# swanhong/matrix-fhe-lattigo

Hardware: AMD Instinct MI355X
Metric: forward-NTT/s at N=2^16, 16 RNS limbs; achieved HBM GB/s vs peak (higher is better)
Workload: dtype u64

## Files before the change

### matrix-fhe-lattigo_amd/csrc/engine.hip

```cpp
#include <hip/hip_runtime.h>
#include <cstdio>
#include <cstdarg>
#include <cstring>
#include <vector>
#include <new>
#include "../../include/ringhip.h"
#include "hostmath.hpp"
#include "ntt_kernels.hip.hpp"
#include "vec_kernels.hip.hpp"
#include "stream_kernels.hip.hpp"
#include "ntt_kernels_asm.hip.hpp"
#include "ntt3n_kernels_asm.hip.hpp"
#include "engine_internal.hpp"

static thread_local char g_err[512] = "";
int rh_fail(int code, const char* fmt, ...) {
  va_list ap; va_start(ap, fmt); vsnprintf(g_err, sizeof(g_err), fmt, ap); va_end(ap);
  return code;
}
extern "C" const char* rh_last_error(void) { return g_err; }

static thread_local hipStream_t tl_stream = nullptr;
static thread_local bool tl_has_stream = false;
static thread_local u64* tl_ws = nullptr;
// ... 416 lines not shown
  } else {
    if (phase != 1) {
      if (r->asm_tile && S1 == 0 && r->inv_scale && r->one_pass && phase == 0) {
        if (nt) ntt_inv_onepass_asm<0, true><<<rows, 256, (size_t)LDS_WORDS * 8, st>>>(in, out, r->d_twk_inv + toff, r->d_tw_inv + toff, r->d_lastw + limb0, c, Lrows, Ls, Lso, 1);
        else ntt_inv_onepass_asm<0, false><<<rows, 256, (size_t)LDS_WORDS * 8, st>>>(in, out, r->d_twk_inv + toff, r->d_tw_inv + toff, r->d_lastw + limb0, c, Lrows, Ls, Lso, 1);
        return rh_launch_ok("ntt (N = 4096, inverse)");
      }
      if (r->asm_tile && (S1 > 0 || !r->inv_scale) && nt) ntt_inv_tile_asm<true><<<tiles, 256, 0, st>>>(in, out, r->d_twk_inv + toff, c, Lrows, logN, npoly, Ls, Lso);
      else if (r->asm_tile && (S1 > 0 || !r->inv_scale)) ntt_inv_tile_asm<false><<<tiles, 256, 0, st>>>(in, out, r->d_twk_inv + toff, c, Lrows, logN, npoly, Ls, Lso);
      else ntt_inv_tile<<<tiles, 256, 0, st>>>(in, out, r->d_twk_inv + toff, c, Lrows, logN, (S1 == 0 && r->inv_scale) ? 1 : 0, npoly, Ls, Lso);
    }
    const bool acols = phase != 2 && r->asm_cols && r->asm_tile && r->inv_scale;
    if (S1 == 4 && acols && nt) ntt_inv_cols_asm<4, true><<<dim3(rows * 16), 256, 0, st>>>(out, r->d_tw_inv + toff, r->d_lastw + limb0, c, Lrows, Lso);
    else if (S1 == 3 && acols && nt) ntt_inv_cols_asm<3, true><<<dim3(rows * 16), 256, 0, st>>>(out, r->d_tw_inv + toff, r->d_lastw + limb0, c, Lrows, Lso);
    else if (S1 == 2 && acols && nt) ntt_inv_cols_asm<2, true><<<dim3(rows * 16), 256, 0, st>>>(out, r->d_tw_inv + toff, r->d_lastw + limb0, c, Lrows, Lso);
    else if (S1 == 4 && acols) ntt_inv_cols_asm<4><<<dim3(rows * 16), 256, 0, st>>>(out, r->d_tw_inv + toff, r->d_lastw + limb0, c, Lrows, Lso);
    else if (S1 == 3 && acols) ntt_inv_cols_asm<3><<<dim3(rows * 16), 256, 0, st>>>(out, r->d_tw_inv + toff, r->d_lastw + limb0, c, Lrows, Lso);
    else if (S1 == 2 && acols) ntt_inv_cols_asm<2><<<dim3(rows * 16), 256, 0, st>>>(out, r->d_tw_inv + toff, r->d_lastw + limb0, c, Lrows, Lso);
    else if (S1 > 0 && phase != 2) launch_inv_cols(S1, dim3(rows * 16), st, out, r->d_tw_inv + toff, r->d_lastw + limb0, c, Lrows, logN, r->inv_scale ? 1 : 0, Lso);
  }
  return rh_launch_ok("ntt");
}

template <int S1>
static void launch_fused(rh_ring* r, const u64* in1, u64* out1, unsigned n1, u64* data2, unsigned n2, int npoly2,
                         size_t toff, const LimbConsts* c, int Lrows) {
  const unsigned grid = n1 > n2 ? n1 : n2;
  hipStream_t st = rh_stream(r);
  constexpr bool has_acols = S1 >= 2 && S1 <= 4;
  if constexpr (has_acols) {
    if (r->asm_tile && r->asm_cols) {
      if (r->nt_streams) ntt_fwd_fused_asm<S1, true, true><<<grid, 256, 0, st>>>(in1, out1, n1, data2, n2, npoly2, r->d_tw_fwd + toff, r->d_twk_fwd + toff, c, Lrows, r->logN);
      else ntt_fwd_fused_asm<S1, true, false><<<grid, 256, 0, st>>>(in1, out1, n1, data2, n2, npoly2, r->d_tw_fwd + toff, r->d_twk_fwd + toff, c, Lrows, r->logN);
      return;
    }
  }
  if (r->asm_tile)
    ntt_fwd_fused_asm<S1, false><<<grid, 256, 0, st>>>(in1, out1, n1, data2, n2, npoly2, r->d_tw_fwd + toff, r->d_twk_fwd + toff, c, Lrows, r->logN);
  else
    ntt_fwd_fused<ShoupPolicy, S1><<<grid, 256, 0, st>>>(in1, out1, n1, data2, n2, npoly2, r->d_tw_fwd + toff, r->d_twk_fwd + toff,
                                                      c, Lrows, r->logN, 1);
}

struct NttSeg { const u64* in; u64* out; int npoly; };
static int std_ntt_fwd_pipelined_segs(rh_ring* r, const NttSeg* segs, int nseg, int Lrows, int limb0, int chunk) {
  (void)hipGetLastError();
  const int N = r->N, S1 = r->logN - LT;
  const size_t toff = (size_t)limb0 * N, stride = (size_t)Lrows * N;
  const LimbConsts* c = r->d_consts + limb0;
  std::vector<NttSeg> spans;
  for (int k = 0; k < nseg; ++k)
    for (int p = 0; p < segs[k].npoly; p += chunk)
      spans.push_back(NttSeg{segs[k].in + (size_t)p * stride, segs[k].out + (size_t)p * stride, segs[k].npoly - p < chunk ? segs[k].npoly - p : chunk});
  const int nspans = (int)spans.size();
// ... 3 lines not shown
    const u64* i1 = j < nspans ? spans[j].in : nullptr; u64* o1 = j < nspans ? spans[j].out : nullptr; u64* d2 = j >= 1 ? spans[j - 1].out : nullptr;
    switch (S1) {
      case 1: launch_fused<1>(r, i1, o1, n1, d2, n2, n2p, toff, c, Lrows); break;
      case 2: launch_fused<2>(r, i1, o1, n1, d2, n2, n2p, toff, c, Lrows); break;
      case 3: launch_fused<3>(r, i1, o1, n1, d2, n2, n2p, toff, c, Lrows); break;
      case 4: launch_fused<4>(r, i1, o1, n1, d2, n2, n2p, toff, c, Lrows); break;
      case 5: launch_fused<5>(r, i1, o1, n1, d2, n2, n2p, toff, c, Lrows); break;
    }
  }
  return rh_launch_ok("ntt_fwd_fused");
}
static int std_ntt_fwd_pipelined(rh_ring* r, const u64* in, u64* out, int npoly, int Lrows, int limb0, int chunk) {
  const NttSeg seg{in, out, npoly};
  return std_ntt_fwd_pipelined_segs(r, &seg, 1, Lrows, limb0, chunk);
}

template <int S1>
static void launch_inv_fused(rh_ring* r, const u64* in1, const u64* in1b, u64* out1, unsigned n1, int npoly1, u64* data2, unsigned n2,
                             size_t toff, int limb0, const LimbConsts* c, int Lrows) {
  const unsigned grid = n1 > n2 ? n1 : n2;
  hipStream_t st = rh_stream(r);
  constexpr bool has_acols = S1 >= 2 && S1 <= 4;
  const bool acols = has_acols && r->asm_cols;
  if (in1b) {
    const tw2* lw = r->d_lastw_r + limb0;
    if constexpr (has_acols) {
      if (acols) { ntt_inv_fused_asm<S1, true, true><<<grid, 256, 0, st>>>(in1, in1b, out1, n1, npoly1, data2, n2, r->d_twk_inv + toff, r->d_tw_inv + toff, lw, c, Lrows, r->logN); return; }
    }
    ntt_inv_fused_asm<S1, false, true><<<grid, 256, 0, st>>>(in1, in1b, out1, n1, npoly1, data2, n2, r->d_twk_inv + toff, r->d_tw_inv + toff, lw, c, Lrows, r->logN);
    return;
  }
  const tw2* lw = r->d_lastw + limb0;
  if constexpr (has_acols) {
    if (acols && !r->nt_streams) { ntt_inv_fused_asm<S1, true, false, false><<<grid, 256, 0, st>>>(in1, nullptr, out1, n1, npoly1, data2, n2, r->d_twk_inv + toff, r->d_tw_inv + toff, lw, c, Lrows, r->logN); return; }
    if (acols) { ntt_inv_fused_asm<S1, true, false><<<grid, 256, 0, st>>>(in1, nullptr, out1, n1, npoly1, data2, n2, r->d_twk_inv + toff, r->d_tw_inv + toff, lw, c, Lrows, r->logN); return; }
  }
  ntt_inv_fused_asm<S1, false, false><<<grid, 256, 0, st>>>(in1, nullptr, out1, n1, npoly1, data2, n2, r->d_twk_inv + toff, r->d_tw_inv + toff, lw, c, Lrows, r->logN);
}
static int std_ntt_inv_pipelined(rh_ring* r, const u64* in, u64* out, int npoly, int Lrows, int limb0, int chunk, const u64* in_b = nullptr) {
  (void)hipGetLastError();
  const int N = r->N, S1 = r->logN - LT;
  const size_t toff = (size_t)limb0 * N, stride = (size_t)Lrows * N;
  const LimbConsts* c = (in_b ? r->d_consts_r : r->d_consts) + limb0;
  const int nspans = (npoly + chunk - 1) / chunk;
  for (int j = 0; j <= nspans; ++j) {
    const int p1 = j * chunk, n1p = j < nspans ? ((npoly - p1 < chunk) ? npoly - p1 : chunk) : 0;
    const int p2 = (j - 1) * chunk, n2p = j >= 1 ? ((npoly - p2 < chunk) ? npoly - p2 : chunk) : 0;
    const unsigned n1 = ((unsigned)n1p * Lrows) << S1, n2 = (unsigned)n2p * Lrows * 16;
    const u64* i1 = in + (size_t)p1 * stride; u64* o1 = out + (size_t)p1 * stride; u64* d2 = out + (size_t)p2 * stride;
    const u64* ib = in_b ? in_b + (size_t)p1 * stride : nullptr;
    switch (S1) {
      case 1: launch_inv_fused<1>(r, i1, ib, o1, n1, n1p, d2, n2, toff, limb0, c, Lrows); break;
      case 2: launch_inv_fused<2>(r, i1, ib, o1, n1, n1p, d2, n2, toff, limb0, c, Lrows); break;
      case 3: launch_inv_fused<3>(r, i1, ib, o1, n1, n1p, d2, n2, toff, limb0, c, Lrows); break;
      case 4: launch_inv_fused<4>(r, i1, ib, o1, n1, n1p, d2, n2, toff, limb0, c, Lrows); break;
      case 5: launch_inv_fused<5>(r, i1, ib, o1, n1, n1p, d2, n2, toff, limb0, c, Lrows); break;
// ... 472 lines not shown
  if (npoly < 0) return rh_fail(RH_ERR_ARG, "polymul: npoly < 0");
  if (a == b) return rh_fail(RH_ERR_ARG, "polymul: a and b must be different blocks (both are transformed in place)");
  const int S1 = r->logN - LT;
  if (r->kind != RH_RING_STANDARD || S1 < 1 || S1 > 5 || !r->asm_tile) return rh_fail(RH_ERR_UNSUPPORTED, "polymul: standard rings with 2^13 <= N <= 2^17 and the hand-scheduled tile bodies");
  const int Lrows = level + 1;
  const unsigned rows = (unsigned)npoly * (unsigned)Lrows;
  if (rows == 0) return RH_OK;
  (void)hipSetDevice(r->device);
  hipStream_t st = rh_stream(r);
  int chunk = r->chunk_polys;
  if (chunk < 0) { const int c = r->auto_span_rows / Lrows > 0 ? r->auto_span_rows / Lrows : 1; chunk = npoly > c ? c : 0; }
  if (chunk > 0 && npoly > chunk) {
    (void)hipGetLastError();
    const int nspans = (npoly + chunk - 1) / chunk;
    const size_t stride = (size_t)Lrows * r->N;
    const bool nt = r->nt_streams != 0;
    auto span = [&](int j, int* n) { const int p0 = j * chunk; *n = (j < 0 || j >= nspans) ? 0 : (npoly - p0 < chunk ? npoly - p0 : chunk); return (size_t)(j < 0 ? 0 : p0) * stride; };
    for (int j = 0; j < nspans + 2; ++j) {
      int p1, p2, p3;
      const size_t o1 = span(j, &p1), o2 = span(j - 1, &p2), o3 = span(j - 2, &p3);
      const unsigned n1 = (unsigned)p1 * Lrows * 16, n2 = ((unsigned)p2 * Lrows) << S1, n3 = (unsigned)p3 * Lrows * 16;
      const unsigned grid = n1 > n2 ? (n1 > n3 ? n1 : n3) : (n2 > n3 ? n2 : n3);
      if (!grid) continue;
#define RH_PM_FUSED(S) do { if (nt) ntt_polymul_fused_asm<S, true><<<grid, 256, 0, st>>>(a + o1, b + o1, n1, a + o2, b + o2, out + o2, n2, p2, out + o3, n3, r->d_tw_fwd, r->d_twk_fwd, \
                                                                                          r->d_twk_inv, r->d_tw_inv, r->d_lastw_r, r->d_consts_r, Lrows, r->logN);                          \
                            else ntt_polymul_fused_asm<S, false><<<grid, 256, 0, st>>>(a + o1, b + o1, n1, a + o2, b + o2, out + o2, n2, p2, out + o3, n3, r->d_tw_fwd, r->d_twk_fwd,      \
                                                                                       r->d_twk_inv, r->d_tw_inv, r->d_lastw_r, r->d_consts_r, Lrows, r->logN); } while (0)
      switch (S1) { case 1: RH_PM_FUSED(1); break; case 2: RH_PM_FUSED(2); break; case 3: RH_PM_FUSED(3); break; case 4: RH_PM_FUSED(4); break; default: RH_PM_FUSED(5); break; }
#undef RH_PM_FUSED
    }
    return rh_launch_ok("polymul (pipelined)");
  }
  if (int rc = std_ntt_launch_span(r, a, a, npoly, Lrows, 0, false, false, 1)) return rc;
  if (int rc = std_ntt_launch_span(r, b, b, npoly, Lrows, 0, false, false, 1)) return rc;
  (void)hipGetLastError();
  if (rh_stream_grid(r, rows).nt) ntt_polymul_tile_asm<true><<<rows << S1, 256, 0, st>>>(a, b, out, r->d_twk_fwd, r->d_twk_inv, r->d_consts_r, Lrows, r->logN, npoly);
  else ntt_polymul_tile_asm<false><<<rows << S1, 256, 0, st>>>(a, b, out, r->d_twk_fwd, r->d_twk_inv, r->d_consts_r, Lrows, r->logN, npoly);
  const bool nt = rh_stream_grid(r, rows).nt;
  if (S1 >= 2 && S1 <= 4 && r->asm_cols) {
#define RH_PM_COLS(S) do { if (nt) ntt_inv_cols_asm<S, true><<<dim3(rows * 16), 256, 0, st>>>(out, r->d_tw_inv, r->d_lastw_r, r->d_consts_r, Lrows, 0); \
                           else ntt_inv_cols_asm<S, false><<<dim3(rows * 16), 256, 0, st>>>(out, r->d_tw_inv, r->d_lastw_r, r->d_consts_r, Lrows, 0); } while (0)
    if (S1 == 4) RH_PM_COLS(4); else if (S1 == 3) RH_PM_COLS(3); else RH_PM_COLS(2);
#undef RH_PM_COLS
  } else launch_inv_cols(S1, dim3(rows * 16), st, out, r->d_tw_inv, r->d_lastw_r, r->d_consts_r, Lrows, r->logN, 1);
  return rh_launch_ok("polymul");
}

// ... 21 lines not shown
  return rh_rescale_reserve(r, npoly);
}

extern "C" int rh_ring_set_tuning(rh_ring* r, const char* key, long value) {
  if (!r || !key) return rh_fail(RH_ERR_ARG, "set_tuning: null argument");
  if (!strcmp(key, "chunk_polys")) { r->chunk_polys = (int)value; return RH_OK; }
  if (!strcmp(key, "asm_tile")) { r->asm_tile = value != 0; return RH_OK; }
  if (!strcmp(key, "auto_span_rows")) { if (value < 1) return rh_fail(RH_ERR_ARG, "auto_span_rows must be >= 1"); r->auto_span_rows = (int)value; return RH_OK; }
  if (!strcmp(key, "fuse_submul")) { r->fuse_submul = (int)value; return RH_OK; }
  if (!strcmp(key, "digit_pipeline")) { r->digit_pipeline = (int)value; return RH_OK; }
  if (!strcmp(key, "fuse_ci")) { r->fuse_ci = (int)value; return RH_OK; }
  if (!strcmp(key, "perm_inv_shape")) { r->perm_inv_shape = (int)value; return RH_OK; }
  if (!strcmp(key, "perm_fwd_shape")) { r->perm_fwd_shape = (int)value; return RH_OK; }
  if (!strcmp(key, "fuse3n")) { r->fuse3n = (int)value; return RH_OK; }
  if (!strcmp(key, "ntt3n_block_order")) {
    if (r->kind != RH_RING_3N) return rh_fail(RH_ERR_ARG, "ntt3n_block_order: not a 3N ring");
    r->block_order3n = value != 0;
    return RH_OK;
  }
  if (!strcmp(key, "asm_cols")) { r->asm_cols = (int)value; return RH_OK; }
  if (!strcmp(key, "ks_small_rows")) { if (value < 0) return rh_fail(RH_ERR_ARG, "ks_small_rows must be >= 0"); r->ks_small_rows = (int)value; return RH_OK; }
  if (!strcmp(key, "pair_submul")) { r->pair_submul = value != 0; return RH_OK; }
  if (!strcmp(key, "one_pass")) { r->one_pass = value != 0; return RH_OK; }
  if (!strcmp(key, "nt_streams")) {
    if (value < 0 || value > 2) return rh_fail(RH_ERR_ARG, "nt_streams must be 0, 1 or 2 (got %ld)", value);
    r->nt_streams = (int)value; if (r->kind == RH_RING_3N) rh_ring3n_set_nt_streams(r, (int)value); return RH_OK;
  }
  return rh_fail(RH_ERR_ARG, "set_tuning: unknown key %s", key);
}

static int slot_acquire(rh_ring* r, RhHostSlot** out) {
  {
    std::lock_guard<std::mutex> lk(r->slot_mu);
    if (!r->free_slots.empty()) { *out = r->free_slots.back(); r->free_slots.pop_back(); return RH_OK; }
  }
  RhHostSlot* sl = new (std::nothrow) RhHostSlot();
  if (!sl) return rh_fail(RH_ERR_NOMEM, "out of host memory");
  sl->words = (size_t)r->N * (r->kind == RH_RING_3N ? 2 : 1);
  if (hipStreamCreateWithFlags(&sl->stream, hipStreamNonBlocking) != hipSuccess) { delete sl; return rh_fail(RH_ERR_DEVICE, "hipStreamCreate failed"); }
  if (hipMalloc((void**)&sl->buf, sl->words * 8) != hipSuccess) { (void)hipStreamDestroy(sl->stream); delete sl; return rh_fail(RH_ERR_NOMEM, "hipMalloc(host-limb scratch) failed"); }
  std::lock_guard<std::mutex> lk(r->slot_mu);
  r->all_slots.push_back(sl);
  *out = sl;
  return RH_OK;
}
static void slot_release(rh_ring* r, RhHostSlot* sl) {
// ... 250 lines not shown
```

### matrix-fhe-lattigo_amd/csrc/engine_internal.hpp

```cpp
#pragma once
#include <hip/hip_runtime.h>
#include <vector>
#include <mutex>
#include <atomic>
#include <cstdint>
#include "../../include/ringhip.h"
#include "ring_types.hip.hpp"

#define RH_MAX_LIMBS 64

int rh_fail(int code, const char* fmt, ...);

inline bool rh_nt_policy(int nt_streams, size_t bytes, size_t threshold) { return nt_streams == 2 || (nt_streams == 1 && bytes >= threshold); }

struct rh_ring3n_state;
struct CiFold { tw2 f, b; };

struct rh_ring {
  int device = 0, kind = 0, N = 0, logN = 0, L = 0;
  hipStream_t stream = nullptr;
  std::vector<uint64_t> moduli, mred, bred, ninv, roots_fwd, roots_bwd, omega3n;
  std::vector<LimbConsts> hconsts;
  LimbConsts* d_consts = nullptr;
  tw2* d_tw_fwd = nullptr;
// ... 12 lines not shown
  std::vector<struct RhPolySlot*> free_poly_slots, all_poly_slots;
  std::recursive_mutex mu;
  rh_ring3n_state* s3n = nullptr;
  std::vector<void*> rescale_tables;
  u64* d_rs[2] = {nullptr, nullptr}; size_t rs_words[2] = {0, 0};
  u64* d_rows = nullptr; size_t rows_words = 0;
  std::atomic<long> stats_rows_direct{0}, stats_rows_compacted{0};
  int fuse_submul = 1;
  int fuse_ci = 1;
  int digit_pipeline = 1;
  int perm_fwd_shape = 44;
  int perm_inv_shape = 44;
  int fuse3n = 1;
  int block_order3n = 0;
  int asm_cols = 1;
  bool asm_tile = true;
  bool inv_scale = true;
  int auto_span_rows = 2048;
  int ks_small_rows = 512;
  bool pair_submul = true;
  bool one_pass = true;
  bool one_pass_ready = false;
  int nt_streams = 1;
  int chunk_polys = -1;
};

int rh_launch_ok(const char* what);
struct RhStreamGrid { dim3 grid; int nt; };
unsigned rh_stream_chunks(const rh_ring* r);
RhStreamGrid rh_stream_grid(const rh_ring* r, unsigned rows);
inline RhStreamGrid rh_stream_begin(const rh_ring* r, unsigned rows) {
  (void)hipSetDevice(r->device);
  (void)hipGetLastError();
  return rh_stream_grid(r, rows);
}
int rh_scheme_args(const rh_ring* r, int level, int npoly, unsigned kinds, int n_multiple, const char* who);
int rh_comps3(const void* in0, const void* in1, const void* in2, const void* out0, const void* out1, const void* out2, const char* who);
struct RhScalars { u64 a[RH_MAX_LIMBS]; u64 b[RH_MAX_LIMBS]; };
int rh_pack_scalars(const rh_ring* r, int level, const u64* a, const u64* b, bool mont, RhScalars* s, const char* who, const char* noun = "scalar");

struct RhHostSlot { hipStream_t stream = nullptr; u64* buf = nullptr; size_t words = 0; };
hipStream_t rh_stream(const rh_ring* r);
u64* rh_ws_override(size_t words);
struct RhCallScope {
  RhCallScope(hipStream_t st, u64* ws = nullptr, size_t ws_words = 0);
  ~RhCallScope();
// ... 16 lines not shown
int rh_std_ntt_fwd_blocks_small(rh_ring* r, u64* data, size_t block_stride, int nblocks, int Ls, const int* gap0, const int* gap_len,
                                rh_ring* r2, u64* data2, size_t block_stride2, int nblocks2, int Ls2, int npoly, bool lazy_out);
bool rh_can_intt_limb_strided(const rh_ring* r);
int rh_std_intt_limb_strided(rh_ring* r, const u64* in, int in_rows, int limb, u64* out, int npoly);
bool rh_can_fuse_submul(const rh_ring* r);
int rh_std_ntt_submul_launch(rh_ring* r, u64* buf, int npoly, int Lrows, int limb0, const u64* y, int y_rows, u64* out, int out_rows,
                             const u64* scalars_host, bool cols_done = false, const u64* z = nullptr, int z_rows = 0);
int rh_std_ntt_submul_launch_pair(rh_ring* r, u64* buf, int npoly, int Lrows, const u64* y0, const u64* y1, int y_rows, u64* out0, u64* out1, int out_rows,
                                  const u64* scalars_host, const u64* z0, const u64* z1, int z_rows);
int rh_std_ntt_expand_cols_launch(rh_ring* r, const u64* tmp, u64* buf, int npoly, int Lrows, const void* table_dev, int mode, u64 qL);
int rh_vec_launch(rh_ring* r, int opcode, const u64* p1, const u64* p2, u64* p3, int npoly, int Lrows, int limb0,
                  const u64* s0, const u64* s1, int rows1 = 0, int rows2 = 0, int rows3 = 0, int half = 0);
int rh_std_intt_rows(rh_ring* r, const u64* in, int in_rows, u64* out, int out_rows, int npoly, int Lrows);
int rh_std_upload_tables(rh_ring* r, const std::vector<tw2>& fs, const std::vector<tw2>& is, const std::vector<u64>* mont,
                         const std::vector<tw2>& lastw);
int rh_upload_consts(rh_ring* r, const std::vector<LimbConsts>& hc);
void rh_rescale_teardown(rh_ring* r);
int rh_rescale_reserve(rh_ring* r, int npoly);
int rh_ring3n_reserve(rh_ring* r, int npoly);
void rh_3n_launch_layer(bool inverse, int S1, unsigned nblocks, hipStream_t st, const u64* in, u64* out, const N3Layer& a, int nt_streams);
int rh_ring3n_setup(rh_ring* r, std::vector<LimbConsts>& hc);
void rh_ring3n_teardown(rh_ring* r);
void rh_ring3n_set_nt_streams(rh_ring* r, int policy);
int rh_ring3n_ntt_launch(rh_ring* r, const u64* in, u64* out, int npoly, int Lrows, int limb0, bool inverse, bool block_order = false);
int rh_ring3n_reorder_launch(rh_ring* r, const u64* in, u64* out, int npoly, int Lrows, bool to_reference);

struct rh_bext;
rh_ring* rh_bext_ringQ(rh_bext* be);
rh_ring* rh_bext_ringP(rh_bext* be);
int rh_bext_scratch(rh_bext* be, int which, size_t words, u64** out);
std::recursive_mutex& rh_bext_mutex(rh_bext* be);
struct RhBextGuard {
  std::unique_lock<std::recursive_mutex> lk; RhCallScope sc;
  explicit RhBextGuard(rh_bext* be) : lk(rh_bext_mutex(be)), sc(rh_stream(rh_bext_ringQ(be))) {}
};
int rh_bext_moddown_ntt_add(rh_bext* be, int levelQ, int levelP, const u64* p1Q, const u64* p1P, u64* p2Q, int npoly, const u64* addend);
int rh_bext_moddown_ntt_pair(rh_bext* be, int levelQ, int levelP, const u64* q0, const u64* q1, const u64* p1P, u64* out0, u64* out1,
                             int npoly, const u64* add0, const u64* add1);
```

### matrix-fhe-lattigo_amd/csrc/ntt3n.hip

```cpp
#include <hip/hip_runtime.h>
#include <vector>
#include <cstring>
#include "engine_internal.hpp"
#include "hostmath.hpp"

struct rh_ring3n_state {
  int a = 0, b = 0, nb = 0, n2 = 0, log_n2 = 0;
  rh_ring* sub = nullptr;
  Limb3N* d_l3 = nullptr;
  tw2* d_r3_fwd = nullptr;
  tw2* d_r3_inv = nullptr;
  std::vector<int> r3_off;
  int r3_stride = 0;
  int* d_rank = nullptr;
  int* d_block_of_rank = nullptr;
  u64* d_tmp = nullptr; size_t tmp_words = 0;
};

RH_DEV u64 add4(u64 x, u64 y, u64 q4) { return csub(x + y, q4); }
RH_DEV u64 sub4(u64 x, u64 y, u64 q4) { return csub(x + q4 - y, q4); }

__global__ void __launch_bounds__(256)
ntt3n_split_fwd(const u64* in, u64* out, int N, const Limb3N* __restrict__ l3, const LimbConsts* __restrict__ consts, int L) {
  const u32 row = blockIdx.x, limb = row % (u32)L;
// ... 558 lines not shown
      ntt3n_perm_inv<<<dim3(rows, chunks(N)), 256, 0, st>>>(in, tmp, N, nb, s->log_n2, s->d_block_of_rank);
    const int S1sub = s->sub ? s->log_n2 - 12 : 0;
    const bool fuse = s->b == 1 && s->sub && r->fuse3n && S1sub >= 1 && S1sub <= 3;
    if (s->sub) {
      if (int rc = rh_std_ntt_launch(s->sub, tmp, tmp, npoly, Lrows * nb, limb0 * nb, true, false, fuse ? 2 : 0)) return rc;
    }
    if (fuse) {
      const tw2* stw = s->sub->d_tw_inv + ((size_t)limb0 * nb << s->log_n2);
      const dim3 g(rows * 16);
      launch_cols_post_inv(r, S1sub, g, st, tmp, out, N, r3i + s->r3_off[1], s->r3_stride, l3, c, Lrows, stw, s->log_n2);
    } else if (s->b == 1) {
      ntt3n_post_b1_inv<<<dim3(rows, chunks(N / 6)), 256, 0, st>>>(tmp, out, N, r3i + s->r3_off[1], s->r3_stride, l3, c, Lrows);
    } else {
      int cnt = nb / 3, step = s->n2;
      for (int l = s->b; l >= 1; --l, cnt /= 3, step *= 3)
        ntt3n_radix3_inv<<<dim3(rows, chunks(cnt * step)), 256, 0, st>>>(tmp, N, step, cnt, r3i + s->r3_off[l], s->r3_stride, l3, c, Lrows);
      ntt3n_split_inv<<<dim3(rows, chunks(N / 2)), 256, 0, st>>>(tmp, out, N, l3, c, Lrows);
    }
  }
  return rh_launch_ok("3N transform");
}

void rh_ring3n_set_nt_streams(rh_ring* r, int policy) { if (r->s3n && r->s3n->sub) r->s3n->sub->nt_streams = policy; }

int rh_ring3n_reserve(rh_ring* r, int npoly) { return ensure_tmp(r->s3n, (size_t)npoly * r->L * r->N); }
```

### matrix-fhe-lattigo_amd/csrc/ntt_kernels.hip.hpp

```cpp
#pragma once
#include "modarith.hip.hpp"

#include "ring_types.hip.hpp"

struct ShoupPolicy {
  typedef tw2 tw_t;
  u64 q, nq, q4;
  RH_DEV void init(const LimbConsts& c) { q = c.q; nq = c.nq; q4 = 4 * c.q; }
  RH_DEV void fwd(u64& U, u64& V, const tw_t& w, bool ) const {
    u64 u = csub(U, q4);
    u64 X = shoup_mul_acc(V, w.w, w.wp, nq, u);
    V = ((u << 1) + q4) - X;
    U = X;
  }
  RH_DEV void inv(u64& U, u64& V, const tw_t& w) const {
    u64 d = U + q4 - V;
    U = csub(U + V, q4);
    V = shoup_mul(d, w.w, w.wp, nq);
  }
  RH_DEV u64 fwd_final(u64 x, bool canonical) const { return canonical ? canon8(x, q) : x; }
};

struct MontPolicy {
  typedef u64 tw_t;
// ... 261 lines not shown
  const RescaleLimb l = T[limb];
  ShoupPolicy p; p.init(consts[limb]);
  u64 x[R];
#pragma unroll
  for (int k = 0; k < R; ++k) {
    u64 t = tmp[((size_t)poly << logN) + col + ((size_t)k << LT)];
    if (mode == 1) t = cred(t + ((qL - 1) >> 1), qL) + l.s;
    x[k] = bred_add(t, l.q, l.bred0);
  }
#pragma unroll
  for (int s = 0; s < S1; ++s) {
    const int h = R >> (s + 1);
#pragma unroll
    for (int g = 0; g < (1 << s); ++g) {
      tw2 w = tw[(1 << s) + g];
#pragma unroll
      for (int e = 0; e < h; ++e) p.fwd(x[g * 2 * h + e], x[g * 2 * h + e + h], w, false);
    }
  }
#pragma unroll
  for (int k = 0; k < R; ++k) out[base + ((size_t)k << LT)] = x[k];
}

template <class P, int S1>
__global__ void __launch_bounds__(256)
ntt_fwd_fused(const u64* in1, u64* out1, unsigned n1, u64* data2, unsigned n2, int npoly2,
              const typename P::tw_t* __restrict__ twn, const typename P::tw_t* __restrict__ twk,
              const LimbConsts* __restrict__ consts, int L, int logN, int canonical) {
  __shared__ u64 lds[LDS_WORDS];
  if (blockIdx.x < n1) fwd_cols_body<P, S1>(blockIdx.x, in1, out1, twn, consts, L, logN);
  if (blockIdx.x < n2) fwd_tile_body<P>(lds, blockIdx.x, data2, data2, twk, consts, L, logN, canonical, npoly2, L);
}

template <int S1>
RH_DEV void inv_cols_body(const u32 b, u64* data, const tw2* __restrict__ twn, const tw2* __restrict__ lastw,
                          const LimbConsts* __restrict__ consts, int L, int logN, int scale, int Ls = 0) {
  constexpr int R = 1 << S1;
  const u32 limb = b % (u32)L;
  const u32 r = b / (u32)L;
  const u32 cb = r & 15;
  const u32 poly = r >> 4;
  const size_t base = (((size_t)poly * (Ls ? Ls : L) + limb) << logN) + cb * 256 + threadIdx.x;
  const tw2* tw = twn + ((size_t)limb << logN);
  const LimbConsts c = consts[limb];
  ShoupPolicy p; p.init(c);
  u64 x[R];
// ... 116 lines not shown
```

### matrix-fhe-lattigo_amd/csrc/ntt_kernels_asm.hip.hpp

```cpp
#pragma once
#include "ring_types.hip.hpp"
#include "ntt_kernels.hip.hpp"
#include "ntt_tile_asm.inc"
#include "ntt_ci_asm.inc"


template <bool LAZY = false, bool NT = false>
RH_DEV void fwd_tile_asm_body(u64* lds, const u32 b, const u64* in, u64* out, const tw2* __restrict__ twk,
                              const LimbConsts* __restrict__ consts, int L, int logN, int npoly, int Ls = 0, u32 gap0 = 0, u32 gap_len = 0, int Lso = 0) {
  if (Ls == 0) Ls = L;
  if (Lso == 0) Lso = Ls;
  const u32 lrow = b % (u32)L;
  const u32 limb = lrow + (lrow >= gap0 ? gap_len : 0u);
  const u32 r = b / (u32)L;
  const u32 poly = r % (u32)npoly;
  const u32 tile = r / (u32)npoly;
  const size_t base = (((size_t)poly * Ls + limb) << logN) + ((size_t)tile << LT);
  const u64 pin = uni64((u64)(size_t)(in + base));
  const u64 pout = uni64((u64)(size_t)(out + (((size_t)poly * Lso + limb) << logN) + ((size_t)tile << LT)));
  const u64 tw = uni64((u64)(size_t)(twk + ((size_t)limb << logN) + ((size_t)tile << LT)));
  const u64 q = uni64(consts[limb].q);
  const u64 nq = (u64)0 - q, nq2 = (u64)0 - 2 * q, nq4 = (u64)0 - 4 * q, q4 = 4 * q;
  const u32 lds_off = uni32((u32)(size_t)lds);
  const u32 tid = threadIdx.x;
// ... 106 lines not shown
  const u64 q = uni64(consts[limb].q);
  const u64 sw = uni64(sc.w[limb]), sp = uni64(sc.wp[limb]);
  const u64 nq = (u64)0 - q, nq2 = (u64)0 - 2 * q, nq4 = (u64)0 - 4 * q, q4 = 4 * q, q2 = 2 * q;
  const u32 lds_off = uni32((u32)(size_t)lds);
  const u32 tid = threadIdx.x;
#define RH_SUBMUL_ADD_ASM(BODY)                                                                                                      \
  asm volatile(BODY : : [tid] "v"(tid), [lds] "s"(lds_off), [pin] "s"(pin), [pout] "s"(pout), [py] "s"(py), [pz] "s"(pz), [tw] "s"(tw),     \
               [twlo] "s"((u32)(size_t)tw), [twhi] "s"((u32)((size_t)tw >> 32)), [nq0] "s"((u32)nq), [nq1] "s"((u32)(nq >> 32)),            \
               [nq] "s"(nq), [nq2] "s"(nq2), [nq4] "s"(nq4), [q4] "s"(q4), [q2] "s"(q2), [sw0] "s"((u32)sw), [sw1] "s"((u32)(sw >> 32)),    \
               [sp0] "s"((u32)sp), [sp1] "s"((u32)(sp >> 32)) : NTT_TILE_ASM_CLOBBERS)
#define RH_SUBMUL_ASM(BODY)                                                                                                          \
  asm volatile(BODY : : [tid] "v"(tid), [lds] "s"(lds_off), [pin] "s"(pin), [pout] "s"(pout), [py] "s"(py), [tw] "s"(tw),                   \
               [twlo] "s"((u32)(size_t)tw), [twhi] "s"((u32)((size_t)tw >> 32)), [nq0] "s"((u32)nq), [nq1] "s"((u32)(nq >> 32)),            \
               [nq] "s"(nq), [nq2] "s"(nq2), [nq4] "s"(nq4), [q4] "s"(q4), [q2] "s"(q2), [sw0] "s"((u32)sw), [sw1] "s"((u32)(sw >> 32)),    \
               [sp0] "s"((u32)sp), [sp1] "s"((u32)(sp >> 32)) : NTT_TILE_ASM_CLOBBERS)
  if constexpr (ADD && NT) RH_SUBMUL_ADD_ASM(NTT_TILE_SUBMUL_ADD_ASM_BODY_NT);
  else if constexpr (ADD) RH_SUBMUL_ADD_ASM(NTT_TILE_SUBMUL_ADD_ASM_BODY);
  else if constexpr (NT) RH_SUBMUL_ASM(NTT_TILE_SUBMUL_ASM_BODY_NT);
  else RH_SUBMUL_ASM(NTT_TILE_SUBMUL_ASM_BODY);
#undef RH_SUBMUL_ADD_ASM
#undef RH_SUBMUL_ASM
}

template <int S1, bool ASMCOLS = false, bool NT = true>
__global__ void __launch_bounds__(256)
ntt_fwd_fused_asm(const u64* in1, u64* out1, unsigned n1, u64* data2, unsigned n2, int npoly2,
                  const tw2* __restrict__ twn, const tw2* __restrict__ twk, const LimbConsts* __restrict__ consts, int L, int logN) {
  __shared__ u64 lds[LDS_WORDS];
  if (blockIdx.x < n1) fwd_cols_best<S1, ASMCOLS, NT>(blockIdx.x, in1, out1, twn, consts, L, logN);
  if (blockIdx.x < n2) fwd_tile_asm_body<false, NT>(lds, blockIdx.x, data2, data2, twk, consts, L, logN, npoly2);
}

struct GapRows { int L, Ls; u32 gap0, gap_len; };
template <int S1, bool LAZY, bool NT>
__global__ void __launch_bounds__(256)
ntt_fwd_fused_gap_asm(u64* data1, unsigned n1, GapRows g1, u64* data2, unsigned n2, int npoly2, GapRows g2,
                      const tw2* __restrict__ twn, const tw2* __restrict__ twk, const LimbConsts* __restrict__ consts) {
  __shared__ u64 lds[LDS_WORDS];
  if (blockIdx.x < n1) fwd_cols_asm_body<S1, NT>(blockIdx.x, data1, data1, twn, consts, g1.L, g1.Ls, g1.gap0, g1.gap_len);
  if (blockIdx.x < n2) fwd_tile_asm_body<LAZY, NT>(lds, blockIdx.x, data2, data2, twk, consts, g2.L, LT + S1, npoly2, g2.Ls, g2.gap0, g2.gap_len);
}

struct GapBlocks { int L[8]; u32 gap0[8], gap_len[8]; int Ls; };
struct BlockSet { u64* data; size_t stride; const tw2* tw; const LimbConsts* consts; GapBlocks g; int nblocks; };
template <int S1>
__global__ void __launch_bounds__(256)
ntt_fwd_cols_blocks_asm(BlockSet a, BlockSet b, int npoly) {
  const bool first = blockIdx.y < (unsigned)a.nblocks;
  const u32 y = first ? blockIdx.y : blockIdx.y - (unsigned)a.nblocks;
  const GapBlocks& g = first ? a.g : b.g;
  const int L = g.L[y];
// ... 109 lines not shown
  const u64 pin = uni64((u64)(size_t)(a + base)), pin2 = uni64((u64)(size_t)(b2 + base)), pout = uni64((u64)(size_t)(out + base));
  const u64 tw = uni64((u64)(size_t)(twk_fwd + toff)), twi = uni64((u64)(size_t)(twk_inv + toff));
  const u64 q = uni64(consts[limb].q), qinv = uni64(consts[limb].qinv);
  const u64 nq = (u64)0 - q, nq2 = (u64)0 - 2 * q, nq4 = (u64)0 - 4 * q, q4 = 4 * q;
  const u32 lds_off = uni32((u32)(size_t)lds);
  const u32 tid = threadIdx.x;
#define RH_TILE_POLYMUL_ASM(BODY)                                                                                                          \
  asm volatile(BODY : : [tid] "v"(tid), [lds] "s"(lds_off), [pin] "s"(pin), [pin2] "s"(pin2), [pout] "s"(pout), [tw] "s"(tw),               \
               [twlo] "s"((u32)(size_t)tw), [twhi] "s"((u32)((size_t)tw >> 32)), [twi] "s"(twi), [twilo] "s"((u32)(size_t)twi),            \
               [twihi] "s"((u32)((size_t)twi >> 32)), [nq0] "s"((u32)nq), [nq1] "s"((u32)(nq >> 32)), [nq] "s"(nq), [nq2] "s"(nq2),       \
               [nq4] "s"(nq4), [q4] "s"(q4), [q] "s"(q), [q0] "s"((u32)q), [q1] "s"((u32)(q >> 32)), [qi0] "s"((u32)qinv),                 \
               [qi1] "s"((u32)(qinv >> 32)) : NTT_TILE_POLYMUL_ASM_CLOBBERS)
  if constexpr (NT) RH_TILE_POLYMUL_ASM(NTT_TILE_POLYMUL_ASM_BODY_NT);
  else RH_TILE_POLYMUL_ASM(NTT_TILE_POLYMUL_ASM_BODY);
#undef RH_TILE_POLYMUL_ASM
}
template <bool NT = false>
__global__ void __launch_bounds__(256)
ntt_polymul_tile_asm(const u64* a, const u64* b2, u64* out, const tw2* __restrict__ twk_fwd, const tw2* __restrict__ twk_inv,
                     const LimbConsts* __restrict__ consts, int L, int logN, int npoly) {
  __shared__ u64 lds[LDS_WORDS];
  polymul_tile_asm_body<NT>(lds, blockIdx.x, a, b2, out, twk_fwd, twk_inv, consts, L, logN, npoly);
}
template <int S1, bool NT>
__global__ void __launch_bounds__(256)
ntt_polymul_fused_asm(u64* a1, u64* b1, unsigned n1, const u64* a2, const u64* b2, u64* out2, unsigned n2, int npoly2, u64* out3, unsigned n3,
                      const tw2* __restrict__ twn_f, const tw2* __restrict__ twk_f, const tw2* __restrict__ twk_i, const tw2* __restrict__ twn_i,
                      const tw2* __restrict__ lastw_r, const LimbConsts* __restrict__ consts_r, int L, int logN) {
  __shared__ u64 lds[LDS_WORDS];
  const u32 b = blockIdx.x;
  if (b < n1) {
    fwd_cols_best<S1, true, NT>(b, a1, a1, twn_f, consts_r, L, logN);
    fwd_cols_best<S1, true, NT>(b, b1, b1, twn_f, consts_r, L, logN);
  }
  if (b < n2) polymul_tile_asm_body<NT>(lds, b, a2, b2, out2, twk_f, twk_i, consts_r, L, logN, npoly2);
  if (b < n3) {
    if constexpr (has_asm_cols(S1)) inv_cols_asm_body<S1, NT>(b, out3, twn_i, lastw_r, consts_r, L);
    else inv_cols_body<S1>(b, out3, twn_i, lastw_r, consts_r, L, logN, 1);
  }
}

template <int S1, bool ASMCOLS = false, bool MUL = false, bool NT = true>
__global__ void __launch_bounds__(256)
ntt_inv_fused_asm(const u64* in1, const u64* in1b, u64* out1, unsigned n1, int npoly1, u64* data2, unsigned n2,
                  const tw2* __restrict__ twk, const tw2* __restrict__ twn, const tw2* __restrict__ lastw,
                  const LimbConsts* __restrict__ consts, int L, int logN) {
  __shared__ u64 lds[LDS_WORDS];
  if (blockIdx.x < n2) {
    if constexpr (has_asm_cols(S1) && ASMCOLS) inv_cols_asm_body<S1, NT>(blockIdx.x, data2, twn, lastw, consts, L);
    else inv_cols_body<S1>(blockIdx.x, data2, twn, lastw, consts, L, logN, 1);
  }
  if (blockIdx.x < n1) inv_tile_asm_body<MUL, NT>(lds, blockIdx.x, in1, in1b, out1, twk, consts, L, logN, npoly1);
}

struct CiFoldTw { tw2 f, b; };
template <int S1, bool INV>
RH_DEV void cols_ci_asm_body(const u32 b, const u64* in, u64* out, const tw2* __restrict__ twn, const tw2* __restrict__ lastw,
                             const CiFoldTw* __restrict__ fold, const LimbConsts* __restrict__ consts, int L) {
  static_assert(has_asm_cols(S1), "asm column stages exist for S1 = 2..4");
  constexpr int logN = LT + S1;
  const u32 limb = b % (u32)L, rr = b / (u32)L, g = rr & 7;
  const size_t row = ((size_t)(rr >> 3) * L + limb) << logN;
  const size_t offa = row + 256 * g + 1, offb = row + 256 * (15 - g);
  const u64 pina = uni64((u64)(size_t)(in + offa)), pinb = uni64((u64)(size_t)(in + offb));
  const u64 pouta = uni64((u64)(size_t)(out + offa)), poutb = uni64((u64)(size_t)(out + offb));
  const u64 tw = uni64((u64)(size_t)(twn + ((size_t)limb << logN)));
  const u64 q = uni64(consts[limb].q);
  const u64 nq = (u64)0 - q, nq2 = (u64)0 - 2 * q, nq4 = (u64)0 - 4 * q, q4 = 4 * q;
  const tw2 F = INV ? fold[limb].b : fold[limb].f;
  const u64 fw = uni64(F.w), fp = uni64(F.wp);
// ... 250 lines not shown
```

Before: 146,000.

## Spread column-stage units across tile-sized grid in fused NTT kernels

When a fused kernel's column-stage unit count differs from its tile count, the launch grid shrinks to roughly the tile count, with a floor of one eighth of the column units. Each block then loops over a contiguous range of column units before doing at most one tile. This replaces many short-lived blocks that do only column work with fewer blocks that each do more, aiming to balance work per block and cut block scheduling overhead. The cost is lower parallelism and possible tail imbalance. The behaviour is controlled by a new fused_spread knob, which is on by default.

Result: no change. 146,000 (median of 2 runs) (-0.0%).

```diff
diff --git a/matrix-fhe-lattigo_amd/csrc/engine.hip b/matrix-fhe-lattigo_amd/csrc/engine.hip
--- a/matrix-fhe-lattigo_amd/csrc/engine.hip
+++ b/matrix-fhe-lattigo_amd/csrc/engine.hip
@@ -462,6 +462,13 @@
   return rh_launch_ok("ntt");
 }
 
+struct FusedShape { unsigned grid; bool spread; };
+static FusedShape fused_shape(const rh_ring* r, unsigned n_tile, unsigned n_a, unsigned n_b = 0) {
+  const unsigned m = n_a > n_b ? n_a : n_b, all = m > n_tile ? m : n_tile;
+  if (!r->fused_spread || !n_tile || ((!n_a || n_a == n_tile) && (!n_b || n_b == n_tile))) return {all, false};
+  const unsigned least = (m + 7) / 8;
+  return {n_tile > least ? n_tile : least, true};
+}
 template <int S1>
 static void launch_fused(rh_ring* r, const u64* in1, u64* out1, unsigned n1, u64* data2, unsigned n2, int npoly2,
                          size_t toff, const LimbConsts* c, int Lrows) {
@@ -470,6 +477,12 @@
   constexpr bool has_acols = S1 >= 2 && S1 <= 4;
   if constexpr (has_acols) {
     if (r->asm_tile && r->asm_cols) {
+      const FusedShape fs = fused_shape(r, n2, n1);
+      if (fs.spread) {
+        if (r->nt_streams) ntt_fwd_fused_asm<S1, true, true, true><<<fs.grid, 256, 0, st>>>(in1, out1, n1, data2, n2, npoly2, r->d_tw_fwd + toff, r->d_twk_fwd + toff, c, Lrows, r->logN);
+        else ntt_fwd_fused_asm<S1, true, false, true><<<fs.grid, 256, 0, st>>>(in1, out1, n1, data2, n2, npoly2, r->d_tw_fwd + toff, r->d_twk_fwd + toff, c, Lrows, r->logN);
+        return;
+      }
       if (r->nt_streams) ntt_fwd_fused_asm<S1, true, true><<<grid, 256, 0, st>>>(in1, out1, n1, data2, n2, npoly2, r->d_tw_fwd + toff, r->d_twk_fwd + toff, c, Lrows, r->logN);
       else ntt_fwd_fused_asm<S1, true, false><<<grid, 256, 0, st>>>(in1, out1, n1, data2, n2, npoly2, r->d_tw_fwd + toff, r->d_twk_fwd + toff, c, Lrows, r->logN);
       return;
@@ -519,9 +532,11 @@
   hipStream_t st = rh_stream(r);
   constexpr bool has_acols = S1 >= 2 && S1 <= 4;
   const bool acols = has_acols && r->asm_cols;
+  const FusedShape fs = fused_shape(r, n1, n2);
   if (in1b) {
     const tw2* lw = r->d_lastw_r + limb0;
     if constexpr (has_acols) {
+      if (acols && fs.spread) { ntt_inv_fused_asm<S1, true, true, true, true><<<fs.grid, 256, 0, st>>>(in1, in1b, out1, n1, npoly1, data2, n2, r->d_twk_inv + toff, r->d_tw_inv + toff, lw, c, Lrows, r->logN); return; }
       if (acols) { ntt_inv_fused_asm<S1, true, true><<<grid, 256, 0, st>>>(in1, in1b, out1, n1, npoly1, data2, n2, r->d_twk_inv + toff, r->d_tw_inv + toff, lw, c, Lrows, r->logN); return; }
     }
     ntt_inv_fused_asm<S1, false, true><<<grid, 256, 0, st>>>(in1, in1b, out1, n1, npoly1, data2, n2, r->d_twk_inv + toff, r->d_tw_inv + toff, lw, c, Lrows, r->logN);
@@ -529,6 +544,8 @@
   }
   const tw2* lw = r->d_lastw + limb0;
   if constexpr (has_acols) {
+    if (acols && fs.spread && !r->nt_streams) { ntt_inv_fused_asm<S1, true, false, false, true><<<fs.grid, 256, 0, st>>>(in1, nullptr, out1, n1, npoly1, data2, n2, r->d_twk_inv + toff, r->d_tw_inv + toff, lw, c, Lrows, r->logN); return; }
+    if (acols && fs.spread) { ntt_inv_fused_asm<S1, true, false, true, true><<<fs.grid, 256, 0, st>>>(in1, nullptr, out1, n1, npoly1, data2, n2, r->d_twk_inv + toff, r->d_tw_inv + toff, lw, c, Lrows, r->logN); return; }
     if (acols && !r->nt_streams) { ntt_inv_fused_asm<S1, true, false, false><<<grid, 256, 0, st>>>(in1, nullptr, out1, n1, npoly1, data2, n2, r->d_twk_inv + toff, r->d_tw_inv + toff, lw, c, Lrows, r->logN); return; }
     if (acols) { ntt_inv_fused_asm<S1, true, false><<<grid, 256, 0, st>>>(in1, nullptr, out1, n1, npoly1, data2, n2, r->d_twk_inv + toff, r->d_tw_inv + toff, lw, c, Lrows, r->logN); return; }
   }
@@ -1047,7 +1064,12 @@
       const unsigned n1 = (unsigned)p1 * Lrows * 16, n2 = ((unsigned)p2 * Lrows) << S1, n3 = (unsigned)p3 * Lrows * 16;
       const unsigned grid = n1 > n2 ? (n1 > n3 ? n1 : n3) : (n2 > n3 ? n2 : n3);
       if (!grid) continue;
-#define RH_PM_FUSED(S) do { if (nt) ntt_polymul_fused_asm<S, true><<<grid, 256, 0, st>>>(a + o1, b + o1, n1, a + o2, b + o2, out + o2, n2, p2, out + o3, n3, r->d_tw_fwd, r->d_twk_fwd, \
+      const FusedShape fs = fused_shape(r, n2, n1, n3);
+#define RH_PM_FUSED(S) do { if (fs.spread && nt) ntt_polymul_fused_asm<S, true, true><<<fs.grid, 256, 0, st>>>(a + o1, b + o1, n1, a + o2, b + o2, out + o2, n2, p2, out + o3, n3, r->d_tw_fwd, r->d_twk_fwd, \
+                                                                                                       r->d_twk_inv, r->d_tw_inv, r->d_lastw_r, r->d_consts_r, Lrows, r->logN);             \
+                            else if (fs.spread) ntt_polymul_fused_asm<S, false, true><<<fs.grid, 256, 0, st>>>(a + o1, b + o1, n1, a + o2, b + o2, out + o2, n2, p2, out + o3, n3, r->d_tw_fwd, r->d_twk_fwd, \
+                                                                                                       r->d_twk_inv, r->d_tw_inv, r->d_lastw_r, r->d_consts_r, Lrows, r->logN);             \
+                            else if (nt) ntt_polymul_fused_asm<S, true><<<grid, 256, 0, st>>>(a + o1, b + o1, n1, a + o2, b + o2, out + o2, n2, p2, out + o3, n3, r->d_tw_fwd, r->d_twk_fwd, \
                                                                                           r->d_twk_inv, r->d_tw_inv, r->d_lastw_r, r->d_consts_r, Lrows, r->logN);                          \
                             else ntt_polymul_fused_asm<S, false><<<grid, 256, 0, st>>>(a + o1, b + o1, n1, a + o2, b + o2, out + o2, n2, p2, out + o3, n3, r->d_tw_fwd, r->d_twk_fwd,      \
                                                                                        r->d_twk_inv, r->d_tw_inv, r->d_lastw_r, r->d_consts_r, Lrows, r->logN); } while (0)
@@ -1115,6 +1137,10 @@
   if (!strcmp(key, "ks_small_rows")) { if (value < 0) return rh_fail(RH_ERR_ARG, "ks_small_rows must be >= 0"); r->ks_small_rows = (int)value; return RH_OK; }
   if (!strcmp(key, "pair_submul")) { r->pair_submul = value != 0; return RH_OK; }
   if (!strcmp(key, "one_pass")) { r->one_pass = value != 0; return RH_OK; }
+  if (!strcmp(key, "fused_spread")) {
+    if (value < 0 || value > 1) return rh_fail(RH_ERR_ARG, "fused_spread must be 0 or 1 (got %ld)", value);
+    r->fused_spread = (int)value; if (r->kind == RH_RING_3N) rh_ring3n_set_fused_spread(r, (int)value); return RH_OK;
+  }
   if (!strcmp(key, "nt_streams")) {
     if (value < 0 || value > 2) return rh_fail(RH_ERR_ARG, "nt_streams must be 0, 1 or 2 (got %ld)", value);
     r->nt_streams = (int)value; if (r->kind == RH_RING_3N) rh_ring3n_set_nt_streams(r, (int)value); return RH_OK;
diff --git a/matrix-fhe-lattigo_amd/csrc/engine_internal.hpp b/matrix-fhe-lattigo_amd/csrc/engine_internal.hpp
--- a/matrix-fhe-lattigo_amd/csrc/engine_internal.hpp
+++ b/matrix-fhe-lattigo_amd/csrc/engine_internal.hpp
@@ -58,6 +58,7 @@
   bool one_pass = true;
   bool one_pass_ready = false;
   int nt_streams = 1;
+  int fused_spread = 1;
   int chunk_polys = -1;
 };
 
@@ -120,6 +121,7 @@
 int rh_ring3n_setup(rh_ring* r, std::vector<LimbConsts>& hc);
 void rh_ring3n_teardown(rh_ring* r);
 void rh_ring3n_set_nt_streams(rh_ring* r, int policy);
+void rh_ring3n_set_fused_spread(rh_ring* r, int spread);
 int rh_ring3n_ntt_launch(rh_ring* r, const u64* in, u64* out, int npoly, int Lrows, int limb0, bool inverse, bool block_order = false);
 int rh_ring3n_reorder_launch(rh_ring* r, const u64* in, u64* out, int npoly, int Lrows, bool to_reference);
 
diff --git a/matrix-fhe-lattigo_amd/csrc/ntt3n.hip b/matrix-fhe-lattigo_amd/csrc/ntt3n.hip
--- a/matrix-fhe-lattigo_amd/csrc/ntt3n.hip
+++ b/matrix-fhe-lattigo_amd/csrc/ntt3n.hip
@@ -604,5 +604,6 @@
 }
 
 void rh_ring3n_set_nt_streams(rh_ring* r, int policy) { if (r->s3n && r->s3n->sub) r->s3n->sub->nt_streams = policy; }
+void rh_ring3n_set_fused_spread(rh_ring* r, int spread) { if (r->s3n && r->s3n->sub) r->s3n->sub->fused_spread = spread; }
 
 int rh_ring3n_reserve(rh_ring* r, int npoly) { return ensure_tmp(r->s3n, (size_t)npoly * r->L * r->N); }
diff --git a/matrix-fhe-lattigo_amd/csrc/ntt_kernels.hip.hpp b/matrix-fhe-lattigo_amd/csrc/ntt_kernels.hip.hpp
--- a/matrix-fhe-lattigo_amd/csrc/ntt_kernels.hip.hpp
+++ b/matrix-fhe-lattigo_amd/csrc/ntt_kernels.hip.hpp
@@ -307,6 +307,12 @@
   for (int k = 0; k < R; ++k) out[base + ((size_t)k << LT)] = x[k];
 }
 
+RH_DEV u32 fused_div(const u64 p, const u32 G) { return (p >> 32) == 0 ? (u32)p / G : (u32)(p / G); }
+RH_DEV void fused_units(const u32 n, u32& lo, u32& hi) {
+  const u32 b = blockIdx.x, G = gridDim.x;
+  if (n == G) { lo = b; hi = b + 1; return; }
+  lo = fused_div((u64)b * n, G); hi = fused_div((u64)(b + 1) * n, G);
+}
 template <class P, int S1>
 __global__ void __launch_bounds__(256)
 ntt_fwd_fused(const u64* in1, u64* out1, unsigned n1, u64* data2, unsigned n2, int npoly2,
diff --git a/matrix-fhe-lattigo_amd/csrc/ntt_kernels_asm.hip.hpp b/matrix-fhe-lattigo_amd/csrc/ntt_kernels_asm.hip.hpp
--- a/matrix-fhe-lattigo_amd/csrc/ntt_kernels_asm.hip.hpp
+++ b/matrix-fhe-lattigo_amd/csrc/ntt_kernels_asm.hip.hpp
@@ -152,11 +152,21 @@
 #undef RH_SUBMUL_ASM
 }
 
-template <int S1, bool ASMCOLS = false, bool NT = true>
+template <int S1, bool ASMCOLS = false, bool NT = true, bool SPREAD = false>
 __global__ void __launch_bounds__(256)
 ntt_fwd_fused_asm(const u64* in1, u64* out1, unsigned n1, u64* data2, unsigned n2, int npoly2,
                   const tw2* __restrict__ twn, const tw2* __restrict__ twk, const LimbConsts* __restrict__ consts, int L, int logN) {
   __shared__ u64 lds[LDS_WORDS];
+  if constexpr (SPREAD) {
+    static_assert(has_asm_cols(S1) && ASMCOLS, "the unit loop goes around the hand-scheduled column stages only");
+    u32 lo, hi;
+    fused_units(n1, lo, hi);
+#pragma nounroll
+    for (u32 u = lo; u < hi; ++u) fwd_cols_asm_body<S1, NT>(u, in1, out1, twn, consts, L);
+    fused_units(n2, lo, hi);
+    if (lo < hi) fwd_tile_asm_body<false, NT>(lds, lo, data2, data2, twk, consts, L, logN, npoly2);
+    return;
+  }
   if (blockIdx.x < n1) fwd_cols_best<S1, ASMCOLS, NT>(blockIdx.x, in1, out1, twn, consts, L, logN);
   if (blockIdx.x < n2) fwd_tile_asm_body<false, NT>(lds, blockIdx.x, data2, data2, twk, consts, L, logN, npoly2);
 }
@@ -312,12 +322,30 @@
   __shared__ u64 lds[LDS_WORDS];
   polymul_tile_asm_body<NT>(lds, blockIdx.x, a, b2, out, twk_fwd, twk_inv, consts, L, logN, npoly);
 }
-template <int S1, bool NT>
+template <int S1, bool NT, bool SPREAD = false>
 __global__ void __launch_bounds__(256)
 ntt_polymul_fused_asm(u64* a1, u64* b1, unsigned n1, const u64* a2, const u64* b2, u64* out2, unsigned n2, int npoly2, u64* out3, unsigned n3,
                       const tw2* __restrict__ twn_f, const tw2* __restrict__ twk_f, const tw2* __restrict__ twk_i, const tw2* __restrict__ twn_i,
                       const tw2* __restrict__ lastw_r, const LimbConsts* __restrict__ consts_r, int L, int logN) {
   __shared__ u64 lds[LDS_WORDS];
+  if constexpr (SPREAD) {
+    u32 lo, hi;
+    fused_units(n1, lo, hi);
+#pragma nounroll
+    for (u32 u = lo; u < hi; ++u) {
+      fwd_cols_best<S1, true, NT>(u, a1, a1, twn_f, consts_r, L, logN);
+      fwd_cols_best<S1, true, NT>(u, b1, b1, twn_f, consts_r, L, logN);
+    }
+    fused_units(n2, lo, hi);
+    if (lo < hi) polymul_tile_asm_body<NT>(lds, lo, a2, b2, out2, twk_f, twk_i, consts_r, L, logN, npoly2);
+    fused_units(n3, lo, hi);
+#pragma nounroll
+    for (u32 u = lo; u < hi; ++u) {
+      if constexpr (has_asm_cols(S1)) inv_cols_asm_body<S1, NT>(u, out3, twn_i, lastw_r, consts_r, L);
+      else inv_cols_body<S1>(u, out3, twn_i, lastw_r, consts_r, L, logN, 1);
+    }
+    return;
+  }
   const u32 b = blockIdx.x;
   if (b < n1) {
     fwd_cols_best<S1, true, NT>(b, a1, a1, twn_f, consts_r, L, logN);
@@ -330,12 +358,22 @@
   }
 }
 
-template <int S1, bool ASMCOLS = false, bool MUL = false, bool NT = true>
+template <int S1, bool ASMCOLS = false, bool MUL = false, bool NT = true, bool SPREAD = false>
 __global__ void __launch_bounds__(256)
 ntt_inv_fused_asm(const u64* in1, const u64* in1b, u64* out1, unsigned n1, int npoly1, u64* data2, unsigned n2,
                   const tw2* __restrict__ twk, const tw2* __restrict__ twn, const tw2* __restrict__ lastw,
                   const LimbConsts* __restrict__ consts, int L, int logN) {
   __shared__ u64 lds[LDS_WORDS];
+  if constexpr (SPREAD) {
+    static_assert(has_asm_cols(S1) && ASMCOLS, "the unit loop goes around the hand-scheduled column stages only");
+    u32 lo, hi;
+    fused_units(n2, lo, hi);
+#pragma nounroll
+    for (u32 u = lo; u < hi; ++u) inv_cols_asm_body<S1, NT>(u, data2, twn, lastw, consts, L);
+    fused_units(n1, lo, hi);
+    if (lo < hi) inv_tile_asm_body<MUL, NT>(lds, lo, in1, in1b, out1, twk, consts, L, logN, npoly1);
+    return;
+  }
   if (blockIdx.x < n2) {
     if constexpr (has_asm_cols(S1) && ASMCOLS) inv_cols_asm_body<S1, NT>(blockIdx.x, data2, twn, lastw, consts, L);
     else inv_cols_body<S1>(blockIdx.x, data2, twn, lastw, consts, L, logN, 1);
```
